# TeemoCaption/FDDM-asr

Hardware: AMD Instinct MI355X
Metric: train-step utterances/sec (10 s @16 kHz, seq_len 256) at 1/2/4/8 MI355X (higher is better)
Workload: dtype bf16; 1 GPU; fddm_zhTW_base C2: WavLM-base + 6L d512 H8 ff2048 decoder, V=8000, T=200, dropout 0.1, n_step_fd=4; global_batch=32, seq_len=256, parallelism=dp1

## Files before the change

fddm-asr_amd/csrc/gemm256.hip:

```cpp
#include "gemm.h"
#include <type_traits>

namespace fddm {
namespace g256 {

typedef __attribute__((address_space(1))) const void* gptr_t;
typedef __attribute__((address_space(3))) void* lptr_t;
typedef unsigned u32x4_t __attribute__((ext_vector_type(4)));
typedef unsigned u32x2_t __attribute__((ext_vector_type(2)));
typedef int i32x4_t __attribute__((ext_vector_type(4)));

#ifndef G256_GM
#define G256_GM 4
#endif
#ifndef G256_DEFER1
#define G256_DEFER2
#endif
constexpr int BM = 256, BN = 256, HALF = 16384, STAGE = 4 * HALF, LDS_BYTES = 2 * STAGE, GM = G256_GM;
constexpr unsigned SRD_W3 = 0x00020000u;
enum { HA0 = 0, HA1 = 1, HB0 = 2, HB1 = 3 };

__device__ __forceinline__ u32x4_t ds_read128(const unsigned char* p) {
  const unsigned a = (unsigned)(size_t)(lptr_t)(void*)p;
  u32x4_t v;
  asm volatile("ds_read_b128 %0, %1" : "=v"(v) : "v"(a) : "memory");
  return v;
}

template <int OFF>
__device__ __forceinline__ u32x4_t ds_read128_at(unsigned a) {
  u32x4_t v;
  asm volatile("ds_read_b128 %0, %1 offset:%2" : "=v"(v) : "v"(a), "n"(OFF) : "memory");
  return v;
}
template <int V> using IC = std::integral_constant<int, V>;

template <int N> __device__ __forceinline__ void vmcnt() {
  asm volatile("s_waitcnt vmcnt(%0)" ::"n"(N < 63 ? N : 63) : "memory");
}

__device__ __forceinline__ void store16(const u32x4_t& d, const i32x4_t& srd, int voff, int soff) {
#ifdef G256_NOSTORE
  if (soff == -1)
#endif
  asm volatile("buffer_store_dwordx4 %0, %1, %2, %3 offen\n\ts_nop 1" ::"v"(d), "v"(voff), "s"(srd), "s"(soff)
               : "memory");
}
__device__ __forceinline__ f32x4_t load16(const i32x4_t& srd, int voff, int soff) {
  f32x4_t v;
  asm volatile("buffer_load_dwordx4 %0, %1, %2, %3 offen" : "=&v"(v) : "v"(voff), "s"(srd), "s"(soff) : "memory");
  return v;
}
__device__ __forceinline__ u32x2_t load8(const i32x4_t& srd, int voff, int soff) {
  u32x2_t v;
  asm volatile("buffer_load_dwordx2 %0, %1, %2, %3 offen" : "=&v"(v) : "v"(voff), "s"(srd), "s"(soff) : "memory");
  return v;
}
constexpr int DG_D = 2;
constexpr int dgelu_wait(int i) {
  return i < DG_D ? 4 * (DG_D - 1 - i) + 6 * i : 2 * (DG_D - 1) + 4 * (DG_D - 1 < 7 - i ? DG_D - 1 : 7 - i);
}
__device__ __forceinline__ void dgelu_vmcnt(int i) {
  switch (i) {
    case 0: vmcnt<dgelu_wait(0)>(); break;
    case 1: vmcnt<dgelu_wait(1)>(); break;
    case 2: vmcnt<dgelu_wait(2)>(); break;
    case 3: vmcnt<dgelu_wait(3)>(); break;
    case 4: vmcnt<dgelu_wait(4)>(); break;
    case 5: vmcnt<dgelu_wait(5)>(); break;
    case 6: vmcnt<dgelu_wait(6)>(); break;
    default: vmcnt<dgelu_wait(7)>(); break;
  }
}
__device__ __forceinline__ i32x4_t make_srd(const void* base) {
  const unsigned long a = (unsigned long)base;
  return i32x4_t{(int)(unsigned)a, (int)(unsigned)(a >> 32), 0x7fffffff, (int)SRD_W3};
}

__device__ __forceinline__ void bar() {
  __builtin_amdgcn_sched_barrier(0);
  __builtin_amdgcn_s_barrier();
  __builtin_amdgcn_sched_barrier(0);
}

#ifdef G256_STAMPS
__device__ unsigned long long g256_stamps[256 * G256_STAMPS];
#endif

template <int EPI, typename OT, bool CONV>
__global__ void __launch_bounds__(512) gemm256_kernel(GemmArgs g) {
  extern __shared__ __attribute__((aligned(16))) unsigned char smem[];
  const int tid = threadIdx.x, lane = tid & 63;
  const int wid = __builtin_amdgcn_readfirstlane(tid >> 6);
  const int wr = wid >> 2, wc = wid & 3;
  const int fr = lane & 15, fg = lane >> 4;

  const int nN = (int)((g.N + BN - 1) / BN), nM = (int)((g.M + BM - 1) / BM), tiles = nN * nM;
  const int G = gridDim.x, wg = blockIdx.x, x = wg & 7, jx = wg >> 3;
  int Wx = 0;
  for (int y = 0; y < x; ++y) Wx += (G - 1 - y) / 8 + 1;
  const int Px = (G - 1 - x) / 8 + 1;
  const int s0 = (int)((long)tiles * Wx / G), s1 = (int)((long)tiles * (Wx + Px) / G);
  const int nmine = (s1 - s0 > jx) ? (s1 - s0 - jx + Px - 1) / Px : 0;
  if (nmine == 0) return;
  auto coords = [&](int i, int& m0, int& n0) {
    const int s = s0 + jx + min(i, nmine - 1) * Px;
    const int per = GM * nN, grp = s / per, first = grp * GM, gsz = min(GM, nM - first), rr = s - grp * per;
    m0 = min((first + rr % gsz) * BM, (int)g.M - BM);
    n0 = min((rr / gsz) * BN, (int)g.N - BN);
  };

  const __amdgpu_buffer_rsrc_t rA = __builtin_amdgcn_make_buffer_rsrc((void*)g.A, 0, 0x7fffffff, SRD_W3);
  const __amdgpu_buffer_rsrc_t rB = __builtin_amdgcn_make_buffer_rsrc((void*)g.B, 0, 0x7fffffff, SRD_W3);
  const int lda = (int)g.lda, ldb = (int)g.ldb, ldc = (int)g.ldc, Nc = (int)g.N;
  int va[2], vb[2];
#pragma unroll
  for (int i = 0; i < 2; ++i) {
    const int row = (wid * 2 + i) * 8 + (lane >> 3);
    const int c = (lane & 7) ^ ((row >> 1) & 7);
    va[i] = (((row >> 6) * 128 + (row & 63)) * lda + c * 8) * 2;
    vb[i] = (((row >> 5) * 64 + (row & 31)) * ldb + c * 8) * 2;
  }
  int vcc[2][2] = {{0, 0}, {0, 0}}, vcn[2][2] = {{0, 0}, {0, 0}};
  auto conv_rows = [&](int (&v)[2][2], int m0) {
#pragma unroll
    for (int h = 0; h < 2; ++h)
#pragma unroll
      for (int i = 0; i < 2; ++i) {
        const int row = (wid * 2 + i) * 8 + (lane >> 3);
        const int c = (lane & 7) ^ ((row >> 1) & 7);
        const int m = m0 + (row >> 6) * 128 + h * 64 + (row & 63);
        const int b = m / (int)g.Mi, tt = m - b * (int)g.Mi;
        v[h][i] = (b * (int)g.sAb + tt * (int)(g.geo.cstride * g.lda) + c * 8) * 2;
      }
  };
  int pd_v = 0, pd_so = 0;
  lptr_t pd_d = nullptr;
#ifdef G256_DEFER2
  int pd0_v = 0;
  lptr_t pd0_d = nullptr;
#endif
  bool pd_b = false;
  auto issue = [&](int h, int buf, int v0, int v1, int so, bool split = false) {
#ifdef G256_NODMA
    if (so != -12345) return;
#endif
    lptr_t d = (lptr_t)(smem + buf * STAGE + h * HALF + wid * 2048);
    const __amdgpu_buffer_rsrc_t& r = h < 2 ? rA : rB;
#ifdef G256_DEFER2
    if (split) {
      pd0_d = d;
      pd0_v = v0;
    } else
#endif
    __builtin_amdgcn_raw_ptr_buffer_load_lds(r, d, 16, v0, so, 0, 0);
    if (split) {
      pd_d = (lptr_t)((unsigned char*)d + 1024);
      pd_v = v1;
      pd_so = so;
      pd_b = h >= 2;
    } else {
      __builtin_amdgcn_raw_ptr_buffer_load_lds(r, (lptr_t)((unsigned char*)d + 1024), 16, v1, so, 0, 0);
    }
  };
  auto issue_pending = [&]() {
#ifdef G256_NODMA
    if (pd_so != -12345) return;
#endif
    if (pd_b) __builtin_amdgcn_raw_ptr_buffer_load_lds(rB, pd_d, 16, pd_v, pd_so, 0, 0);
    else __builtin_amdgcn_raw_ptr_buffer_load_lds(rA, pd_d, 16, pd_v, pd_so, 0, 0);
  };
  const int nk = (int)(g.K / 64);
  const int cshift = CONV ? __builtin_ctz((unsigned)(g.geo.Cg / 64)) : 0;
  auto koffA = [&](int kt) -> int {
    if (!CONV) return kt * 128;
    return ((kt >> cshift) * lda + (kt & ((1 << cshift) - 1)) * 64) * 2;
  };
  int cm0, cn0, nm0, nn0;
  coords(0, cm0, cn0);
  coords(1, nm0, nn0);
  constexpr bool ACC = EPI == EPI_ACC_F32;
  auto shifts = [&](int i, int m0, int n0, int& dm, int& dn) {
    const int s = s0 + jx + min(i, nmine - 1) * Px;
    const int per = GM * nN, grp = s / per, first = grp * GM, gsz = min(GM, nM - first), rr = s - grp * per;
    dm = (first + rr % gsz) * BM - m0;
    dn = (rr / gsz) * BN - n0;
  };
  int cdm = 0, cdn = 0, ndm = 0, ndn = 0, edm = 0, edn = 0;
  if constexpr (ACC) {
    shifts(0, cm0, cn0, cdm, cdn);
    shifts(1, nm0, nn0, ndm, ndn);
  }
  if (CONV) {
    conv_rows(vcc, cm0);
    conv_rows(vcn, nm0);
  }
  auto issueA = [&](int h, int buf, int kt, int m0, const int (&vc)[2][2], bool split = false) {
    if (CONV) issue(h, buf, vc[h][0], vc[h][1], koffA(kt), split);
    else issue(h, buf, va[0], va[1], m0 * lda * 2 + h * 64 * lda * 2 + koffA(kt), split);
  };
  auto issueB = [&](int h, int buf, int kt, int n0, bool split = false) {
    issue(h, buf, vb[0], vb[1], n0 * ldb * 2 + (h - 2) * 32 * ldb * 2 + kt * 128, split);
  };

  const bool has_bias = g.bias != nullptr;
  unsigned char* bslot = smem + LDS_BYTES + wid * 256;
  auto load_bias = [&](int n0, bool real) {
    const float* src = has_bias ? g.bias + n0 + wc * 64 + lane : (const float*)g.A + lane;
    __builtin_amdgcn_global_load_lds((gptr_t)src, (lptr_t)(real ? bslot : bslot + 2048), 4, 0, 0);
  };
  auto bias_pair = [&](int jb, f32x4_t& v0, f32x4_t& v1) {
    const u32x4_t a = ds_read128(bslot + (jb * 16 + 4 * fg) * 4);
    const u32x4_t b = ds_read128(bslot + ((jb + 1) * 16 + 4 * fg) * 4);
    asm volatile("s_waitcnt lgkmcnt(0)" ::: "memory");
    v0 = __builtin_bit_cast(f32x4_t, a);
    v1 = __builtin_bit_cast(f32x4_t, b);
    asm volatile("" : "+v"(v0), "+v"(v1));
    if (!has_bias) {
      v0 = f32x4_t{0.f, 0.f, 0.f, 0.f};
      v1 = v0;
    }
  };

  const i32x4_t rc = make_srd(g.C);
  const i32x4_t rc2 = make_srd(EPI == EPI_GELU || EPI == EPI_DGELU ? g.C2 : g.C);
  constexpr int ESZ = (int)sizeof(OT);
  constexpr int SPH = sizeof(OT) == 4 ? 16 : (EPI == EPI_GELU ? 16 : 8);
  const int cc = sizeof(OT) == 4 ? 4 * fg : 4 * fg + ((fg & 1) ? 12 : 0);
  const int vst = ((wr * 128 + (fr & ~1)) * ldc + wc * 64 + (fr & 1) * (sizeof(OT) == 4 ? 16 : 32) + cc) * ESZ;
  const bool odd_r = fr & 1;
  const int vld = ((wr * 128 + fr) * ldc + wc * 64 + 4 * fg) * ESZ;
  const int srow = wr * 128 + (fr & ~1), scol = wc * 64 + (fr & 1) * 16 + 4 * fg;

  u32x4_t af[4][2], b0[2][2], b1[2][2];
  f32x4_t acc[8][4];

  auto xchg1 = [&](u32x4_t& x0, u32x4_t& x1) {
#pragma unroll
    for (int e = 0; e < 4; ++e) {
      const unsigned a = x0[e], b = x1[e];
      const unsigned pb = (unsigned)__builtin_amdgcn_mov_dpp((int)b, 0xb1, 0xf, 0xf, false);
      const unsigned pa = (unsigned)__builtin_amdgcn_mov_dpp((int)a, 0xb1, 0xf, 0xf, false);
      x0[e] = odd_r ? pb : a;
      x1[e] = odd_r ? b : pa;
    }
  };
  auto chunk16 = [&](const f32x4_t& a, const f32x4_t& b) -> u32x4_t {
    const auto s0 = __builtin_amdgcn_permlane16_swap(pk_bf16(a[0], a[1]), pk_bf16(b[0], b[1]), false, false);
    const auto s1 = __builtin_amdgcn_permlane16_swap(pk_bf16(a[2], a[3]), pk_bf16(b[2], b[3]), false, false);
    return u32x4_t{s0[0], s1[0], s0[1], s1[1]};
  };
  auto emit_bf16 = [&](const f32x4_t (&v)[4], const i32x4_t& r, int so) {
    u32x4_t x0 = chunk16(v[0], v[1]), x1 = chunk16(v[2], v[3]);
    xchg1(x0, x1);
    store16(x0, r, vst, so);
    store16(x1, r, vst, so + ldc * ESZ);
  };

  auto epi_rows = [&](auto ibc, auto nc, int em0, int en0, bool reseed) {
    constexpr int ib = decltype(ibc)::value, NR = decltype(nc)::value;
    f32x4_t bq[4];
    if constexpr (!ACC) {
      if (reseed) {
        bias_pair(0, bq[0], bq[1]);
        bias_pair(2, bq[2], bq[3]);
      }
    }
    u32x2_t pre[DG_D][4];
    auto load_pre = [&](int i) {
#pragma unroll
      for (int j = 0; j < 4; ++j)
        pre[i % DG_D][j] = load8(rc2, vld, ((em0 + i * 16) * ldc + en0 + j * 16) * ESZ);
    };
    if constexpr (EPI == EPI_DGELU) {
      static_assert(EPI != EPI_DGELU || (ib == 0 && NR == 8), "dgelu_wait counts a whole tile");
#pragma unroll
      for (int i = 0; i < DG_D; ++i) load_pre(i);
    }
#pragma unroll
    for (int i = 0; i < NR; ++i) {
      const int so = ((em0 + (ib + i) * 16) * ldc + en0) * ESZ;
      if constexpr (ACC) {
#pragma unroll
        for (int p = 0; p < 2; ++p) {
          u32x4_t x0 = __builtin_bit_cast(u32x4_t, acc[ib + i][2 * p]);
          u32x4_t x1 = __builtin_bit_cast(u32x4_t, acc[ib + i][2 * p + 1]);
          xchg1(x0, x1);
          const bool cok = scol + 32 * p >= edn;
          const int r = srow + (ib + i) * 16;
          if (cok && r >= edm) store16(x0, rc, vst, so + 32 * p * ESZ);
          if (cok && r + 1 >= edm) store16(x1, rc, vst, so + (ldc + 32 * p) * ESZ);
        }
        if (reseed) {
#pragma unroll
          for (int j = 0; j < 4; ++j)
            acc[ib + i][j] = load16(rc, vld, ((cm0 + (ib + i) * 16) * ldc + cn0 + j * 16) * ESZ);
        }
      } else if constexpr (sizeof(OT) == 4) {
#pragma unroll
        for (int p = 0; p < 2; ++p) {
          u32x4_t x0 = __builtin_bit_cast(u32x4_t, acc[ib + i][2 * p]);
          u32x4_t x1 = __builtin_bit_cast(u32x4_t, acc[ib + i][2 * p + 1]);
          xchg1(x0, x1);
          store16(x0, rc, vst, so + 32 * p * ESZ);
          store16(x1, rc, vst, so + (ldc + 32 * p) * ESZ);
        }
      } else {
        f32x4_t v[4] = {acc[ib + i][0], acc[ib + i][1], acc[ib + i][2], acc[ib + i][3]};
        if constexpr (EPI == EPI_GELU) {
          emit_bf16(v, rc, so);
          const unsigned thr = g.thr16;
#pragma unroll
          for (int j = 0; j < 4; ++j) {
            unsigned keep = 0xfu;
            if (thr) {
              const unsigned m = (unsigned)(em0 + wr * 128 + (ib + i) * 16 + fr);
              const unsigned n = (unsigned)(en0 + wc * 64 + j * 16 + 4 * fg);
              keep = drop_keep4(eff_seed(g.seed, g.seed_off), g.stream, ((uint64_t)m * (uint64_t)Nc + n) >> 2, thr);
            }
#pragma unroll
            for (int e = 0; e < 4; ++e) {
              const float a = gelu_f(v[j][e]);
              v[j][e] = thr ? ((keep >> e) & 1u ? a * g.drop_scale : 0.f) : a;
            }
          }
          emit_bf16(v, rc2, so);
        } else if constexpr (EPI == EPI_DGELU) {
          dgelu_vmcnt(i);
          asm volatile("" : "+v"(pre[i % DG_D][0]), "+v"(pre[i % DG_D][1]), "+v"(pre[i % DG_D][2]), "+v"(pre[i % DG_D][3]));
          const unsigned thr = g.thr16;
#pragma unroll
          for (int j = 0; j < 4; ++j) {
            unsigned keep = 0xfu;
            if (thr) {
              const unsigned m = (unsigned)(em0 + wr * 128 + (ib + i) * 16 + fr);
              const unsigned n = (unsigned)(en0 + wc * 64 + j * 16 + 4 * fg);
              keep = drop_keep4(eff_seed(g.seed, g.seed_off), g.stream, ((uint64_t)m * (uint64_t)Nc + n) >> 2, thr);
            }
            const u32x2_t pu = pre[i % DG_D][j];
            const float pv[4] = {__uint_as_float(pu[0] << 16), __uint_as_float(pu[0] & 0xffff0000u),
                                 __uint_as_float(pu[1] << 16), __uint_as_float(pu[1] & 0xffff0000u)};
#pragma unroll
            for (int e = 0; e < 4; ++e) {
              const float a = v[j][e] * gelu_grad(pv[e]);
              v[j][e] = (keep >> e) & 1u ? (thr ? a * g.drop_scale : a) : 0.f;
            }
          }
          emit_bf16(v, rc, so);
          if (i + DG_D < NR) load_pre(i + DG_D);
        } else {
          if constexpr (EPI == EPI_GELU_ONLY) {
#pragma unroll
            for (int j = 0; j < 4; ++j)
#pragma unroll
              for (int e = 0; e < 4; ++e) v[j][e] = gelu_bf16out(v[j][e]);
          }
          emit_bf16(v, rc, so);
        }
      }
      if constexpr (!ACC) {
        if (reseed) {
#pragma unroll
          for (int j = 0; j < 4; ++j) acc[ib + i][j] = bq[j];
        }
      }
      __builtin_amdgcn_sched_barrier(0);
    }
  };

  const unsigned lds0 = (unsigned)(size_t)(lptr_t)(void*)smem;
  const unsigned aadr[2] = {lds0 + wr * 8192 + swz_kc(fr, fg), lds0 + wr * 8192 + swz_kc(fr, 4 + fg)};
  const unsigned badr[2] = {lds0 + wc * 4096 + swz_kc(fr, fg), lds0 + wc * 4096 + swz_kc(fr, 4 + fg)};
  auto readA = [&](int buf, auto hc) {
    constexpr int h = decltype(hc)::value;
#ifdef G256_NOREAD
    asm volatile("" : "+v"(af[0][0]), "+v"(af[1][0]), "+v"(af[2][0]), "+v"(af[3][0]), "+v"(af[0][1]), "+v"(af[1][1]),
                 "+v"(af[2][1]), "+v"(af[3][1]));
    if (buf >= 0) return;
#endif
#pragma unroll
    for (int s = 0; s < 2; ++s) {
      const unsigned a = aadr[s] + buf * STAGE;
      af[0][s] = ds_read128_at<h * HALF + 0 * 2048>(a);
      af[1][s] = ds_read128_at<h * HALF + 1 * 2048>(a);
      af[2][s] = ds_read128_at<h * HALF + 2 * 2048>(a);
      af[3][s] = ds_read128_at<h * HALF + 3 * 2048>(a);
    }
  };
  auto readB = [&](int buf, auto hc, u32x4_t(&bf)[2][2]) {
    constexpr int h = decltype(hc)::value;
#ifdef G256_NOREAD
    asm volatile("" : "+v"(bf[0][0]), "+v"(bf[1][0]), "+v"(bf[0][1]), "+v"(bf[1][1]));
    if (buf >= 0) return;
#endif
#pragma unroll
    for (int s = 0; s < 2; ++s) {
      const unsigned a = badr[s] + buf * STAGE;
      bf[0][s] = ds_read128_at<h * HALF + 0 * 2048>(a);
      bf[1][s] = ds_read128_at<h * HALF + 1 * 2048>(a);
    }
  };
  auto mma = [&](int ib, int jb, const u32x4_t(&bf)[2][2]) {
    bar();
    asm volatile("s_waitcnt lgkmcnt(0)" ::: "memory");
    __builtin_amdgcn_sched_barrier(0);
    __builtin_amdgcn_s_setprio(1);
#pragma unroll
    for (int i = 0; i < 4; ++i) {
#pragma unroll
      for (int j = 0; j < 2; ++j)
#pragma unroll
        for (int s = 0; s < 2; ++s)
          acc[ib + i][jb + j] = __builtin_amdgcn_mfma_f32_16x16x32_bf16(
              __builtin_bit_cast(bf16x8_t, bf[j][s]), __builtin_bit_cast(bf16x8_t, af[i][s]), acc[ib + i][jb + j], 0, 0,
              0);
#ifdef G256_DEFER2
      if (i == 0) {
        __builtin_amdgcn_sched_barrier(0);
        if (pd_b) __builtin_amdgcn_raw_ptr_buffer_load_lds(rB, pd0_d, 16, pd0_v, pd_so, 0, 0);
        else __builtin_amdgcn_raw_ptr_buffer_load_lds(rA, pd0_d, 16, pd0_v, pd_so, 0, 0);
        __builtin_amdgcn_sched_barrier(0);
      }
      if (i == 2) {
#else
      if (i == 1) {
#endif
        __builtin_amdgcn_sched_barrier(0);
        issue_pending();
        __builtin_amdgcn_sched_barrier(0);
      }
    }
    __builtin_amdgcn_s_setprio(0);
    bar();
  };

  if constexpr (ACC) {
#pragma unroll
    for (int i = 0; i < 8; ++i)
#pragma unroll
      for (int j = 0; j < 4; ++j) acc[i][j] = load16(rc, vld, ((cm0 + i * 16) * ldc + cn0 + j * 16) * ESZ);
  }
  load_bias(cn0, true);
  {
    const int kt1 = 1 % nk;
    const int m1 = nk > 1 ? cm0 : nm0, n1 = nk > 1 ? cn0 : nn0;
    issueA(HA0, 0, 0, cm0, vcc);
    issueB(HB0, 0, 0, cn0);
    issueB(HB1, 0, 0, cn0);
    issueA(HA1, 0, 0, cm0, vcc);
    issueA(HA0, 1, kt1, m1, nk > 1 ? vcc : vcn);
    issueB(HB0, 1, kt1, n1);
  }
  vmcnt<8>();
  bar();
  if constexpr (ACC) {
#pragma unroll
    for (int i = 0; i < 8; ++i)
      asm volatile("" : "+v"(acc[i][0]), "+v"(acc[i][1]), "+v"(acc[i][2]), "+v"(acc[i][3]));
  } else {
#pragma unroll
    for (int jb = 0; jb < 4; jb += 2) {
      f32x4_t v0, v1;
      bias_pair(jb, v0, v1);
#pragma unroll
      for (int i = 0; i < 8; ++i) {
        acc[i][jb] = v0;
        acc[i][jb + 1] = v1;
      }
    }
  }
  readB(0, IC<HB0>{}, b0);
  if (wr == 1) bar();

  int em0 = 0, en0 = 0, kt = 0, ti = 0;
  const int NT = nmine * nk;
  auto wait2 = [&](bool EP, auto n0c, auto nec) {
    if (EP) vmcnt<decltype(nec)::value>();
    else vmcnt<decltype(n0c)::value>();
  };
#ifdef G256_DEFER2
  constexpr int D2 = 1;
#else
  constexpr int D2 = 0;
#endif
  constexpr int EPS = ACC ? 0 : 2 * SPH;
  auto ktile = [&](int T, bool EP) {
    const int bc = T & 1, bn = bc ^ 1;
    const bool n1b = kt == nk - 1, n2 = kt >= nk - 2;
    const int kt1 = n1b ? 0 : kt + 1;
    const int kt2 = n2 ? kt + 2 - nk : kt + 2;
    const int m1 = n1b ? nm0 : cm0, n1 = n1b ? nn0 : cn0;
    const int m2 = n2 ? nm0 : cm0, n2c = n2 ? nn0 : cn0;
    readA(bc, IC<HA0>{});
    load_bias(nn0, n1b);
    issueB(HB1, bn, kt1, n1, true);
    vmcnt<8 - D2>();
    if (EP) epi_rows(IC<0>{}, IC<8>{}, em0, en0, true);
    if constexpr (ACC) {
      if (EP) {
        vmcnt<0>();
#pragma unroll
        for (int i = 0; i < 8; ++i)
          asm volatile("" : "+v"(acc[i][0]), "+v"(acc[i][1]), "+v"(acc[i][2]), "+v"(acc[i][3]));
      }
    }
    mma(0, 0, b0);
    readB(bc, IC<HB1>{}, b1);
    if (CONV) issueA(HA1, bn, kt1, m1, n1b ? vcn : vcc, true);
    else issueA(HA1, bn, kt1, m1, vcc, true);
    wait2(EP, IC<8 - D2>{}, IC<8 - D2 + EPS>{});
    mma(0, 2, b1);
    readA(bc, IC<HA1>{});
    if (CONV) issueA(HA0, bc, kt2, m2, n2 ? vcn : vcc, true);
    else issueA(HA0, bc, kt2, m2, vcc, true);
    wait2(EP, IC<6 - D2>{}, IC<6 - D2 + EPS>{});
    mma(4, 0, b0);
    readB(bn, IC<HB0>{}, b0);
    issueB(HB0, bc, kt2, n2c, true);
    wait2(EP, IC<10 - D2>{}, IC<10 - D2 + EPS>{});
    mma(4, 2, b1);
  };
  auto next_tile = [&]() {
    em0 = cm0;
    en0 = cn0;
    cm0 = nm0;
    cn0 = nn0;
    coords(ti + 2, nm0, nn0);
    if constexpr (ACC) {
      edm = cdm;
      edn = cdn;
      cdm = ndm;
      cdn = ndn;
      shifts(ti + 2, nm0, nn0, ndm, ndn);
    }
    if (CONV) {
#pragma unroll
      for (int h = 0; h < 2; ++h)
#pragma unroll
        for (int i = 0; i < 2; ++i) vcc[h][i] = vcn[h][i];
      conv_rows(vcn, nm0);
    }
    ++ti;
  };
  for (int T = 0; T < NT; ++T) {
    const bool later = ti > 0;
#ifdef G256_STAMPS
    if (tid == 0 && T < G256_STAMPS) g256_stamps[blockIdx.x * G256_STAMPS + T] = __builtin_amdgcn_s_memtime();
#endif
    ktile(T, later && kt == 0);
    if (kt == nk - 1) {
      next_tile();
      kt = 0;
    } else {
      ++kt;
    }
  }
  if (wr == 0) bar();
  epi_rows(IC<0>{}, IC<8>{}, em0, en0, false);
  vmcnt<0>();
}

static int g_grid_cap = 0;

template <int EPI, typename OT, bool CONV>
static int launch(const GemmArgs& g, hipStream_t s) {
  static int ncu = 0;
  if (ncu == 0) {
    int dev = 0;
    if (hipGetDevice(&dev) != hipSuccess ||
        hipDeviceGetAttribute(&ncu, hipDeviceAttributeMultiprocessorCount, dev) != hipSuccess || ncu <= 0)
      ncu = 256;
  }
  const long tiles = gemm256_tiles(g.M, g.N);
#ifdef G256_NOPERSIST
  const long grid = tiles;
#else
  const long cap = (g_grid_cap > 0 && g_grid_cap < ncu) ? g_grid_cap : ncu;
  const long rounds = (tiles + cap - 1) / cap;
  const long need = ((tiles + rounds - 1) / rounds + 7) & ~7L;
  const long grid = tiles < cap ? tiles : (need < cap ? need : cap);
#endif
  hipLaunchKernelGGL((gemm256_kernel<EPI, OT, CONV>), dim3((unsigned)grid), dim3(512), LDS_BYTES + 4096, s, g);
  return (int)hipGetLastError();
}

}

long gemm256_tiles(long M, long N) { return ((M + 255) / 256) * ((N + 255) / 256); }

bool gemm256_ok(const GemmArgs& g, int epi, int out_dtype, bool conv) {
  if (g.K % 64 || g.K < 128 || g.M <= 0 || g.N <= 0 || g.N % 8 || g.lda % 8 || g.ldb % 8 || g.ldc % 8) return false;
  if (g.alpha != 1.f) return false;
  if ((((uintptr_t)g.A) | ((uintptr_t)g.B) | ((uintptr_t)g.C) | ((uintptr_t)g.C2) | ((uintptr_t)g.bias)) & 15)
    return false;
  if (g.M < 256 || g.N < 256) return false;
  const long aext = conv ? ((g.M / g.Mi) * g.sAb + g.geo.Tin * g.lda) : ((g.M - 1) * g.lda + g.K);
  if (aext * 2 >= (1L << 31) || ((g.N - 1) * g.ldb + g.K) * 2 >= (1L << 31)) return false;
  if (conv && (g.M % g.Mi || g.geo.cstride * g.lda >= (1L << 31))) return false;
  const long esz = out_dtype == FDDM_F32 ? 4 : 2;
  if (((g.M - 1) * g.ldc + g.N) * esz >= (1L << 31)) return false;
  if (conv && (g.geo.cpad != 0 || g.geo.Cg % 64 || ((g.geo.Cg / 64) & (g.geo.Cg / 64 - 1)))) return false;
  if (out_dtype == FDDM_F32) return (epi == EPI_STORE || (epi == EPI_ACC_F32 && !g.bias)) && !conv;
  if (conv) return epi == EPI_STORE || epi == EPI_GELU_ONLY;
  if (epi == EPI_DGELU) return g.C2 != nullptr && g.C2 != g.C;
  return epi == EPI_STORE || epi == EPI_GELU || epi == EPI_GELU_ONLY;
}

int gemm256_launch(const GemmArgs& g, int epi, int out_dtype, bool conv, hipStream_t s) {
  if (!gemm256_ok(g, epi, out_dtype, conv)) return (int)hipErrorInvalidValue;
  if (out_dtype == FDDM_F32)
    return epi == EPI_ACC_F32 ? g256::launch<EPI_ACC_F32, float, false>(g, s) : g256::launch<EPI_STORE, float, false>(g, s);
  if (conv) {
    if (epi == EPI_GELU_ONLY) return g256::launch<EPI_GELU_ONLY, bf16_t, true>(g, s);
    return g256::launch<EPI_STORE, bf16_t, true>(g, s);
  }
  if (epi == EPI_DGELU) return g256::launch<EPI_DGELU, bf16_t, false>(g, s);
  if (epi == EPI_GELU) return g256::launch<EPI_GELU, bf16_t, false>(g, s);
  if (epi == EPI_GELU_ONLY) return g256::launch<EPI_GELU_ONLY, bf16_t, false>(g, s);
  return g256::launch<EPI_STORE, bf16_t, false>(g, s);
}

}

FDDM_API int fddm_gemm_persistent_cap(int cap) {
  const int prev = fddm::g256::g_grid_cap;
  fddm::g256::g_grid_cap = cap > 0 ? (cap & ~7) : 0;
  return prev;
}

#ifdef G256_STAMPS
FDDM_API int fddm_gemm256_stamps(unsigned long long* host, long n) {
  return (int)hipMemcpyFromSymbol(host, HIP_SYMBOL(fddm::g256::g256_stamps), n * sizeof(unsigned long long), 0,
                                  hipMemcpyDeviceToHost);
}
#endif
```

Before: 3505 utterances/s.

## Restructure 256x256 GEMM k-tile into two MFMA phases with interleaved DMA pieces

Merges the four per-k-tile MFMA phases into two larger phases. Each phase covers both B fragment halves, which halves the number of barriers per k-tile. Global-to-LDS buffer loads are split into single pieces and issued through a callback between MFMA groups, replacing the deferred-pending DMA mechanism. The A/B prefetch schedule and vmcnt waits are retuned, and both B halves are now prefetched two stages ahead. The prologue now always prefetches k-tile 1 of the current tile, which may be wrong when K equals 64.

```diff
diff --git a/fddm-asr_amd/csrc/gemm256.hip b/fddm-asr_amd/csrc/gemm256.hip
--- a/fddm-asr_amd/csrc/gemm256.hip
+++ b/fddm-asr_amd/csrc/gemm256.hip
@@ -12,9 +12,6 @@
 
 #ifndef G256_GM
 #define G256_GM 4
-#endif
-#ifndef G256_DEFER1
-#define G256_DEFER2
 #endif
 constexpr int BM = 256, BN = 256, HALF = 16384, STAGE = 4 * HALF, LDS_BYTES = 2 * STAGE, GM = G256_GM;
 constexpr unsigned SRD_W3 = 0x00020000u;
@@ -134,41 +131,13 @@
         v[h][i] = (b * (int)g.sAb + tt * (int)(g.geo.cstride * g.lda) + c * 8) * 2;
       }
   };
-  int pd_v = 0, pd_so = 0;
-  lptr_t pd_d = nullptr;
-#ifdef G256_DEFER2
-  int pd0_v = 0;
-  lptr_t pd0_d = nullptr;
-#endif
-  bool pd_b = false;
-  auto issue = [&](int h, int buf, int v0, int v1, int so, bool split = false) {
+  auto piece = [&](int h, int buf, int p, int v, int so) {
 #ifdef G256_NODMA
     if (so != -12345) return;
 #endif
-    lptr_t d = (lptr_t)(smem + buf * STAGE + h * HALF + wid * 2048);
-    const __amdgpu_buffer_rsrc_t& r = h < 2 ? rA : rB;
-#ifdef G256_DEFER2
-    if (split) {
-      pd0_d = d;
-      pd0_v = v0;
-    } else
-#endif
-    __builtin_amdgcn_raw_ptr_buffer_load_lds(r, d, 16, v0, so, 0, 0);
-    if (split) {
-      pd_d = (lptr_t)((unsigned char*)d + 1024);
-      pd_v = v1;
-      pd_so = so;
-      pd_b = h >= 2;
-    } else {
-      __builtin_amdgcn_raw_ptr_buffer_load_lds(r, (lptr_t)((unsigned char*)d + 1024), 16, v1, so, 0, 0);
-    }
-  };
-  auto issue_pending = [&]() {
-#ifdef G256_NODMA
-    if (pd_so != -12345) return;
-#endif
-    if (pd_b) __builtin_amdgcn_raw_ptr_buffer_load_lds(rB, pd_d, 16, pd_v, pd_so, 0, 0);
-    else __builtin_amdgcn_raw_ptr_buffer_load_lds(rA, pd_d, 16, pd_v, pd_so, 0, 0);
+    lptr_t d = (lptr_t)(smem + buf * STAGE + h * HALF + wid * 2048 + p * 1024);
+    if (h < 2) __builtin_amdgcn_raw_ptr_buffer_load_lds(rA, d, 16, v, so, 0, 0);
+    else __builtin_amdgcn_raw_ptr_buffer_load_lds(rB, d, 16, v, so, 0, 0);
   };
   const int nk = (int)(g.K / 64);
   const int cshift = CONV ? __builtin_ctz((unsigned)(g.geo.Cg / 64)) : 0;
@@ -195,12 +164,20 @@
     conv_rows(vcc, cm0);
     conv_rows(vcn, nm0);
   }
-  auto issueA = [&](int h, int buf, int kt, int m0, const int (&vc)[2][2], bool split = false) {
-    if (CONV) issue(h, buf, vc[h][0], vc[h][1], koffA(kt), split);
-    else issue(h, buf, va[0], va[1], m0 * lda * 2 + h * 64 * lda * 2 + koffA(kt), split);
-  };
-  auto issueB = [&](int h, int buf, int kt, int n0, bool split = false) {
-    issue(h, buf, vb[0], vb[1], n0 * ldb * 2 + (h - 2) * 32 * ldb * 2 + kt * 128, split);
+  auto pieceA = [&](int h, int buf, int kt, int m0, const int (&vc)[2][2], int p) {
+    if (CONV) piece(h, buf, p, vc[h][p], koffA(kt));
+    else piece(h, buf, p, va[p], m0 * lda * 2 + h * 64 * lda * 2 + koffA(kt));
+  };
+  auto pieceB = [&](int h, int buf, int kt, int n0, int p) {
+    piece(h, buf, p, vb[p], n0 * ldb * 2 + (h - 2) * 32 * ldb * 2 + kt * 128);
+  };
+  auto issueA = [&](int h, int buf, int kt, int m0, const int (&vc)[2][2]) {
+    pieceA(h, buf, kt, m0, vc, 0);
+    pieceA(h, buf, kt, m0, vc, 1);
+  };
+  auto issueB = [&](int h, int buf, int kt, int n0) {
+    pieceB(h, buf, kt, n0, 0);
+    pieceB(h, buf, kt, n0, 1);
   };
 
   const bool has_bias = g.bias != nullptr;
@@ -400,7 +377,7 @@
       bf[1][s] = ds_read128_at<h * HALF + 1 * 2048>(a);
     }
   };
-  auto mma = [&](int ib, int jb, const u32x4_t(&bf)[2][2]) {
+  auto mma = [&](int ib, auto&& dma) {
     bar();
     asm volatile("s_waitcnt lgkmcnt(0)" ::: "memory");
     __builtin_amdgcn_sched_barrier(0);
@@ -408,25 +385,17 @@
 #pragma unroll
     for (int i = 0; i < 4; ++i) {
 #pragma unroll
-      for (int j = 0; j < 2; ++j)
-#pragma unroll
-        for (int s = 0; s < 2; ++s)
-          acc[ib + i][jb + j] = __builtin_amdgcn_mfma_f32_16x16x32_bf16(
-              __builtin_bit_cast(bf16x8_t, bf[j][s]), __builtin_bit_cast(bf16x8_t, af[i][s]), acc[ib + i][jb + j], 0, 0,
-              0);
-#ifdef G256_DEFER2
-      if (i == 0) {
+      for (int jp = 0; jp < 2; ++jp) {
+        const u32x4_t(&bf)[2][2] = jp ? b1 : b0;
+#pragma unroll
+        for (int j = 0; j < 2; ++j)
+#pragma unroll
+          for (int s = 0; s < 2; ++s)
+            acc[ib + i][2 * jp + j] = __builtin_amdgcn_mfma_f32_16x16x32_bf16(
+                __builtin_bit_cast(bf16x8_t, bf[j][s]), __builtin_bit_cast(bf16x8_t, af[i][s]), acc[ib + i][2 * jp + j],
+                0, 0, 0);
         __builtin_amdgcn_sched_barrier(0);
-        if (pd_b) __builtin_amdgcn_raw_ptr_buffer_load_lds(rB, pd0_d, 16, pd0_v, pd_so, 0, 0);
-        else __builtin_amdgcn_raw_ptr_buffer_load_lds(rA, pd0_d, 16, pd0_v, pd_so, 0, 0);
-        __builtin_amdgcn_sched_barrier(0);
-      }
-      if (i == 2) {
-#else
-      if (i == 1) {
-#endif
-        __builtin_amdgcn_sched_barrier(0);
-        issue_pending();
+        dma(2 * i + jp);
         __builtin_amdgcn_sched_barrier(0);
       }
     }
@@ -441,16 +410,13 @@
       for (int j = 0; j < 4; ++j) acc[i][j] = load16(rc, vld, ((cm0 + i * 16) * ldc + cn0 + j * 16) * ESZ);
   }
   load_bias(cn0, true);
-  {
-    const int kt1 = 1 % nk;
-    const int m1 = nk > 1 ? cm0 : nm0, n1 = nk > 1 ? cn0 : nn0;
-    issueA(HA0, 0, 0, cm0, vcc);
-    issueB(HB0, 0, 0, cn0);
-    issueB(HB1, 0, 0, cn0);
-    issueA(HA1, 0, 0, cm0, vcc);
-    issueA(HA0, 1, kt1, m1, nk > 1 ? vcc : vcn);
-    issueB(HB0, 1, kt1, n1);
-  }
+  issueA(HA0, 0, 0, cm0, vcc);
+  issueB(HB0, 0, 0, cn0);
+  issueB(HB1, 0, 0, cn0);
+  issueA(HA1, 0, 0, cm0, vcc);
+  issueA(HA0, 1, 1, cm0, vcc);
+  issueB(HB0, 1, 1, cn0);
+  issueB(HB1, 1, 1, cn0);
   vmcnt<8>();
   bar();
   if constexpr (ACC) {
@@ -469,7 +435,6 @@
       }
     }
   }
-  readB(0, IC<HB0>{}, b0);
   if (wr == 1) bar();
 
   int em0 = 0, en0 = 0, kt = 0, ti = 0;
@@ -478,11 +443,6 @@
     if (EP) vmcnt<decltype(nec)::value>();
     else vmcnt<decltype(n0c)::value>();
   };
-#ifdef G256_DEFER2
-  constexpr int D2 = 1;
-#else
-  constexpr int D2 = 0;
-#endif
   constexpr int EPS = ACC ? 0 : 2 * SPH;
   auto ktile = [&](int T, bool EP) {
     const int bc = T & 1, bn = bc ^ 1;
@@ -491,34 +451,40 @@
     const int kt2 = n2 ? kt + 2 - nk : kt + 2;
     const int m1 = n1b ? nm0 : cm0, n1 = n1b ? nn0 : cn0;
     const int m2 = n2 ? nm0 : cm0, n2c = n2 ? nn0 : cn0;
-    readA(bc, IC<HA0>{});
-    load_bias(nn0, n1b);
-    issueB(HB1, bn, kt1, n1, true);
-    vmcnt<8 - D2>();
-    if (EP) epi_rows(IC<0>{}, IC<8>{}, em0, en0, true);
-    if constexpr (ACC) {
-      if (EP) {
+    auto frags1 = [&]() {
+      readA(bc, IC<HA0>{});
+      readB(bc, IC<HB0>{}, b0);
+      readB(bc, IC<HB1>{}, b1);
+    };
+    if (!EP) frags1();
+    vmcnt<6>();
+    if (EP) {
+      epi_rows(IC<0>{}, IC<8>{}, em0, en0, true);
+      frags1();
+      if constexpr (ACC) {
         vmcnt<0>();
 #pragma unroll
         for (int i = 0; i < 8; ++i)
           asm volatile("" : "+v"(acc[i][0]), "+v"(acc[i][1]), "+v"(acc[i][2]), "+v"(acc[i][3]));
       }
     }
-    mma(0, 0, b0);
-    readB(bc, IC<HB1>{}, b1);
-    if (CONV) issueA(HA1, bn, kt1, m1, n1b ? vcn : vcc, true);
-    else issueA(HA1, bn, kt1, m1, vcc, true);
-    wait2(EP, IC<8 - D2>{}, IC<8 - D2 + EPS>{});
-    mma(0, 2, b1);
+    mma(0, [&](int k) {
+      if (k == 0) load_bias(nn0, n1b);
+      if (k == 2 || k == 4) {
+        if (CONV) pieceA(HA1, bn, kt1, m1, n1b ? vcn : vcc, k == 4);
+        else pieceA(HA1, bn, kt1, m1, vcc, k == 4);
+      }
+    });
     readA(bc, IC<HA1>{});
-    if (CONV) issueA(HA0, bc, kt2, m2, n2 ? vcn : vcc, true);
-    else issueA(HA0, bc, kt2, m2, vcc, true);
-    wait2(EP, IC<6 - D2>{}, IC<6 - D2 + EPS>{});
-    mma(4, 0, b0);
-    readB(bn, IC<HB0>{}, b0);
-    issueB(HB0, bc, kt2, n2c, true);
-    wait2(EP, IC<10 - D2>{}, IC<10 - D2 + EPS>{});
-    mma(4, 2, b1);
+    wait2(EP, IC<3>{}, IC<3 + EPS>{});
+    mma(4, [&](int k) {
+      if (k == 0 || k == 1) {
+        if (CONV) pieceA(HA0, bc, kt2, m2, n2 ? vcn : vcc, k);
+        else pieceA(HA0, bc, kt2, m2, vcc, k);
+      }
+      if (k == 2 || k == 3) pieceB(HB0, bc, kt2, n2c, k - 2);
+      if (k == 4 || k == 5) pieceB(HB1, bc, kt2, n2c, k - 4);
+    });
   };
   auto next_tile = [&]() {
     em0 = cm0;
```

Result: no change. 3504 utterances/s (-0.0%).
